# EmbersArc/SCpp

Hardware: AMD Instinct MI355X
Metric: converged SCvx trajectories/sec (RocketQuat, K=50) at 1/2/4/8 MI355X (higher is better)
Workload: dtype f64

## Files before the change

### __graft_entry__.py

```python
import os
import subprocess
import sys

ROOT = os.path.dirname(os.path.abspath(__file__))
CSRC = os.path.join(ROOT, "scpp_amd", "csrc")
HIP_LIB = os.path.join(ROOT, "scpp_amd", "libscpp_hip.so")
HOST_LIB = os.path.join(ROOT, "scpp_amd", "libscpp_host.so")
EMU_LIB = os.path.join(ROOT, "tests", "emu", "libscpp_emu.so")
LQR_LIB = os.path.join(ROOT, "scpp_amd", "libscpp_lqr.so")
LQR_EMU_LIB = os.path.join(ROOT, "tests", "emu", "libscpp_lqr_emu.so")
LQR_SRC = os.path.join(CSRC, "lqr", "scpp_hip_lqr.cpp")
TILE_PROBE_SRC = os.path.join(ROOT, "tests", "tile_probe", "tile_probe.cpp")
TILE_PROBE_LIB = os.path.join(ROOT, "tests", "tile_probe", "libtile_probe.so")
TILE_PROBE_EMU_LIB = os.path.join(ROOT, "tests", "emu", "libtile_probe_emu.so")
SWEEP_PROBE_SRC = os.path.join(ROOT, "tests", "sweep_probe", "sweep_probe.cpp")
SWEEP_PROBE_LIB = os.path.join(ROOT, "tests", "sweep_probe", "libsweep_probe.so")
SWEEP_PROBE_EMU_LIB = os.path.join(ROOT, "tests", "emu", "libsweep_probe_emu.so")
CONE_PROBE_SRC = os.path.join(ROOT, "tests", "cone_probe", "cone_probe.cpp")
CONE_PROBE_LIB = os.path.join(ROOT, "tests", "cone_probe", "libcone_probe.so")
CONE_PROBE_EMU_LIB = os.path.join(ROOT, "tests", "emu", "libcone_probe_emu.so")
PHASE_PROBE_SRC = os.path.join(ROOT, "tests", "phase_probe", "phase_probe.cpp")
PHASE_PROBE_LIB = os.path.join(ROOT, "tests", "phase_probe", "libphase_probe.so")
PHASE_PROBE_MEM_LIB = os.path.join(ROOT, "tests", "phase_probe", "libphase_probe_prevlane_memory.so")
PHASE_PROBE_EMU_LIB = os.path.join(ROOT, "tests", "emu", "libphase_probe_emu.so")
HIP_FP_FLAGS = ["-ffp-contract=on"]


class _BuildLock:

    def __enter__(self):
        import fcntl

        try:
            self.f = open(os.path.join(ROOT, ".build.lock"), "w")
            fcntl.flock(self.f, fcntl.LOCK_EX)
        except OSError:
            self.f = None
        return self

    def __exit__(self, *exc):
        import fcntl

        if self.f is not None:
            fcntl.flock(self.f, fcntl.LOCK_UN)
            self.f.close()
        return False


def _newer(target, sources):
    if not os.path.exists(target):
        return True
    t = os.path.getmtime(target)
    return any(os.path.getmtime(s) > t for s in sources)


def _sources(d, exts):
    out = []
    for base, _, files in os.walk(d):
        out += [os.path.join(base, f) for f in files if f.endswith(exts)]
    return out


def build_hip(force=False):
    srcs = _sources(CSRC, (".h", ".cpp")) + [os.path.join(ROOT, "include", "scpp_hip.h")]
    if force or _newer(HIP_LIB, srcs):
        subprocess.check_call(
            ["hipcc", "--offload-arch=gfx950", "-O3", "-std=c++17", "-fPIC", "-shared", "-x", "hip"] + HIP_FP_FLAGS +
            [os.path.join(CSRC, "scpp_hip.cpp"), "-o", HIP_LIB]
        )
    return HIP_LIB


def build_host(force=False):
    host = os.path.join(ROOT, "scpp_amd", "host")
    if os.path.isdir(host) and os.path.exists(os.path.join(host, "Makefile")):
        with _BuildLock():
            subprocess.check_call(["make", "-s", "-C", host, "all"])


def build_oracle():
    with _BuildLock():
        subprocess.check_call(["make", "-s", "-C", os.path.join(ROOT, "oracle"), "liboracle.so"])


def build_emu(force=False):
    srcs = _sources(CSRC, (".h", ".cpp")) + [os.path.join(ROOT, "tests", "emu", "hip_emu.h")]
    with _BuildLock():
        if force or _newer(EMU_LIB, srcs):
            tmp = EMU_LIB + ".tmp%d" % os.getpid()
            subprocess.check_call(
                ["g++", "-O1", "-std=c++17", "-fPIC", "-DSCPP_HIP_EMU", "-I" + os.path.join(ROOT, "tests", "emu"), "-shared",
                 "-o", tmp, "-x", "c++", os.path.join(CSRC, "scpp_hip.cpp")]
            )
            os.replace(tmp, EMU_LIB)
    return EMU_LIB


def _lqr_sources():
    return _sources(os.path.join(CSRC, "lqr"), (".h", ".cpp")) + [os.path.join(CSRC, f) for f in (
        "common.h", "model_rocketquat.h", "model_lander3dof.h", "model_jacobian_rows.h")] + [os.path.join(ROOT, "include", "scpp_hip_lqr.h")]


def build_lqr(force=False):
    if force or _newer(LQR_LIB, _lqr_sources()):
        subprocess.check_call(
            ["hipcc", "--offload-arch=gfx950", "-O3", "-std=c++17", "-fPIC", "-shared", "-x", "hip"] + HIP_FP_FLAGS + [LQR_SRC, "-o", LQR_LIB]
        )
    return LQR_LIB


def build_lqr_emu(force=False):
    with _BuildLock():
        if force or _newer(LQR_EMU_LIB, _lqr_sources() + [os.path.join(ROOT, "tests", "emu", "hip_emu.h")]):
            tmp = LQR_EMU_LIB + ".tmp%d" % os.getpid()
            subprocess.check_call(
                ["g++", "-O1", "-std=c++17", "-fPIC", "-DSCPP_HIP_EMU", "-I" + os.path.join(ROOT, "tests", "emu"), "-shared",
                 "-o", tmp, "-x", "c++", LQR_SRC]
            )
            os.replace(tmp, LQR_EMU_LIB)
    return LQR_EMU_LIB


def _tile_probe_sources():
    return [TILE_PROBE_SRC] + [os.path.join(CSRC, f) for f in ("tile_engine.h", "ipm_kernel.h", "common.h", "cone_math.h", "constraint_table.h")]


def build_tile_probe(force=False):
    with _BuildLock():
        if force or _newer(TILE_PROBE_LIB, _tile_probe_sources()):
            tmp = TILE_PROBE_LIB + ".tmp%d" % os.getpid()
            subprocess.check_call(
                ["hipcc", "--offload-arch=gfx950", "-O3", "-std=c++17", "-fPIC", "-shared", "-x", "hip"] + HIP_FP_FLAGS + [TILE_PROBE_SRC, "-o", tmp]
            )
            os.replace(tmp, TILE_PROBE_LIB)
    return TILE_PROBE_LIB


def build_tile_probe_emu(force=False):
    with _BuildLock():
        if force or _newer(TILE_PROBE_EMU_LIB, _tile_probe_sources() + [os.path.join(ROOT, "tests", "emu", "hip_emu.h")]):
            tmp = TILE_PROBE_EMU_LIB + ".tmp%d" % os.getpid()
            subprocess.check_call(
                ["g++", "-O1", "-std=c++17", "-fPIC", "-DSCPP_HIP_EMU", "-I" + os.path.join(ROOT, "tests", "emu"), "-shared",
                 "-o", tmp, "-x", "c++", TILE_PROBE_SRC]
            )
            os.replace(tmp, TILE_PROBE_EMU_LIB)
    return TILE_PROBE_EMU_LIB


def _sweep_probe_sources():
    return [SWEEP_PROBE_SRC] + [os.path.join(CSRC, f) for f in ("sweeps.h", "tile_engine.h", "ipm_kernel.h", "common.h", "cone_math.h", "constraint_table.h")]


def build_sweep_probe(force=False):
    with _BuildLock():
        if force or _newer(SWEEP_PROBE_LIB, _sweep_probe_sources()):
            tmp = SWEEP_PROBE_LIB + ".tmp%d" % os.getpid()
            subprocess.check_call(
                ["hipcc", "--offload-arch=gfx950", "-O3", "-std=c++17", "-fPIC", "-shared", "-x", "hip"] + HIP_FP_FLAGS + [SWEEP_PROBE_SRC, "-o", tmp]
            )
            os.replace(tmp, SWEEP_PROBE_LIB)
    return SWEEP_PROBE_LIB


def build_sweep_probe_emu(force=False):
    with _BuildLock():
        if force or _newer(SWEEP_PROBE_EMU_LIB, _sweep_probe_sources() + [os.path.join(ROOT, "tests", "emu", "hip_emu.h")]):
            tmp = SWEEP_PROBE_EMU_LIB + ".tmp%d" % os.getpid()
            subprocess.check_call(
                ["g++", "-O1", "-std=c++17", "-fPIC", "-DSCPP_HIP_EMU", "-I" + os.path.join(ROOT, "tests", "emu"), "-shared",
                 "-o", tmp, "-x", "c++", SWEEP_PROBE_SRC]
            )
            os.replace(tmp, SWEEP_PROBE_EMU_LIB)
    return SWEEP_PROBE_EMU_LIB


def _cone_probe_sources():
    return [CONE_PROBE_SRC] + [os.path.join(CSRC, f) for f in (
        "cone_math.h", "ipm_solve.h", "ipm_kernel.h", "sweeps.h", "tile_engine.h", "common.h", "constraint_table.h")]


def build_cone_probe(force=False):
    with _BuildLock():
        if force or _newer(CONE_PROBE_LIB, _cone_probe_sources()):
            tmp = CONE_PROBE_LIB + ".tmp%d" % os.getpid()
            subprocess.check_call(
                ["hipcc", "--offload-arch=gfx950", "-O3", "-std=c++17", "-fPIC", "-shared", "-x", "hip"] + HIP_FP_FLAGS + [CONE_PROBE_SRC, "-o", tmp]
            )
            os.replace(tmp, CONE_PROBE_LIB)
    return CONE_PROBE_LIB


def build_cone_probe_emu(force=False):
    with _BuildLock():
        if force or _newer(CONE_PROBE_EMU_LIB, _cone_probe_sources() + [os.path.join(ROOT, "tests", "emu", "hip_emu.h")]):
            tmp = CONE_PROBE_EMU_LIB + ".tmp%d" % os.getpid()
            subprocess.check_call(
                ["g++", "-O1", "-std=c++17", "-fPIC", "-DSCPP_HIP_EMU", "-I" + os.path.join(ROOT, "tests", "emu"), "-shared",
                 "-o", tmp, "-x", "c++", CONE_PROBE_SRC]
            )
            os.replace(tmp, CONE_PROBE_EMU_LIB)
    return CONE_PROBE_EMU_LIB


def _phase_probe_sources():
    return [PHASE_PROBE_SRC] + [os.path.join(CSRC, f) for f in (
        "ipm_solve.h", "ipm_kernel.h", "sweeps.h", "tile_engine.h", "common.h", "cone_math.h", "constraint_table.h")]


def _build_phase_probe_hip(lib, defines, force):
    with _BuildLock():
        if force or _newer(lib, _phase_probe_sources()):
            tmp = lib + ".tmp%d" % os.getpid()
            subprocess.check_call(
                ["hipcc", "--offload-arch=gfx950", "-O3", "-std=c++17", "-fPIC", "-shared", "-x", "hip"] + HIP_FP_FLAGS + defines + [PHASE_PROBE_SRC, "-o", tmp]
            )
            os.replace(tmp, lib)
    return lib


def build_phase_probe(force=False):
    return _build_phase_probe_hip(PHASE_PROBE_LIB, [], force)


def build_phase_probe_prevlane_memory(force=False):
    return _build_phase_probe_hip(PHASE_PROBE_MEM_LIB, ["-DRES_PREVLANE_MEMORY=1"], force)


def build_phase_probe_emu(force=False):
    with _BuildLock():
        if force or _newer(PHASE_PROBE_EMU_LIB, _phase_probe_sources() + [os.path.join(ROOT, "tests", "emu", "hip_emu.h")]):
            tmp = PHASE_PROBE_EMU_LIB + ".tmp%d" % os.getpid()
            subprocess.check_call(
                ["g++", "-O1", "-std=c++17", "-fPIC", "-DSCPP_HIP_EMU", "-I" + os.path.join(ROOT, "tests", "emu"), "-shared",
                 "-o", tmp, "-x", "c++", PHASE_PROBE_SRC]
            )
            os.replace(tmp, PHASE_PROBE_EMU_LIB)
    return PHASE_PROBE_EMU_LIB


def build():
    build_hip()
    build_lqr()
    build_host()
    build_oracle()
    build_emu()
    build_lqr_emu()
    build_tile_probe()
    build_tile_probe_emu()
    build_sweep_probe()
    build_sweep_probe_emu()
    build_cone_probe()
    build_cone_probe_emu()
    build_phase_probe()
    build_phase_probe_prevlane_memory()
    build_phase_probe_emu()
    sys.path.insert(0, ROOT)
    import scpp_amd

    scpp_amd.load_library(HIP_LIB)


def smoke():
    sys.path.insert(0, ROOT)
    sys.path.insert(0, os.path.join(ROOT, "tests"))
    import numpy as np
    import scpp_amd
    import oracle_lib

    if not os.path.exists(HIP_LIB):
        build_hip()
    model = scpp_amd.RocketQuat().loadParameters()
    B, K = 4, 50
    x0 = model.randomized_initial_states(B)
    alg = scpp_amd.SCAlgorithm(model, K=K, batch_max=B, device=0, library=os.environ.get("SCPP_HIP_LIBRARY")).initialize()
    alg.solve(x0)
    out = alg.getSolution()
    ref = oracle_lib.sc_batch(K, 20260927, 0, B, nthreads=4, solver=1)
    sx = np.abs(ref["X"]).max(axis=1, keepdims=True)
    su = np.abs(ref["U"]).max(axis=1, keepdims=True)
    relX = float((np.abs(out["X"] - ref["X"]) / np.maximum(sx, 1e-9)).max())
    relU = float((np.abs(out["U"] - ref["U"]) / np.maximum(su, 1e-9)).max())
    assert (out["status"] == 0).all(), out["status"]
    assert (out["sc_iters"] == ref["iters"]).all(), (out["sc_iters"], ref["iters"])
    assert relX < 1e-5 and relU < 1e-5, (relX, relU)
    print(f"smoke ok: relX={relX:.2e} relU={relU:.2e} sc_iters={out['sc_iters'].tolist()} nu={out['nu_norm'].tolist()}")
    alg.ctx.close()
    import lqr_reference

    if not os.path.exists(LQR_LIB):
        build_lqr()
    trk = scpp_amd.LQRTracker(model, out["X"], out["U"], out["sigma"], library=os.environ.get("SCPP_LQR_LIBRARY"))
    assert trk.n_ok == B * K, (trk.n_ok, trk.status)
    Ks = lqr_reference.scipy_gain(0, out["X"][0, 0], out["U"][0, 0], model.flow_params(nondimensionalize=False), trk.Q, trk.R)
    gk = float(np.abs(trk.gains[0, 0] - Ks).max() / np.abs(Ks).max())
    fl = trk.track(x0)
    assert gk < 1e-6 and fl["n_finite"] == B and all(np.isfinite(fl[k]).all() for k in ("x", "u", "err1")), (gk, fl)
    print(f"smoke ok (lqr): {trk.n_ok} gains, node 0 vs scipy {gk:.2e}, {int(fl['steps'].sum())} tracked plant steps, final error / initial error {(fl['err1'] / fl['err0']).round(3).tolist()}")
    trk.close()
    valg = scpp_amd.SCvxAlgorithm(model, K=K, batch_max=4, device=0, library=os.environ.get("SCPP_HIP_LIBRARY")).initialize()
    xs = model.randomized_initial_states(6)
    nconv = valg.solveStream(xs, slots=4, pools=2)
    so = valg.getStreamSolution()
    assert (so["status"] == 0).all() and (so["instance"] == np.arange(6)).all() and nconv == int(so["converged"].sum())
    ov = oracle_lib.SCvx(K=K)
    ov.randomize(20260927, 0)
    ov.set_solver(1)
    assert ov.solve() == 0
    mv = ov.meta()
    Xo, Uo, _ = ov.iterate(-1)
    assert so["converged"][0] == mv["converged"] == 1
    same_path = so["sc_iters"][0] == mv["iterations"] and so["solves"][0] == mv["solves"]
    rx = float(np.abs(so["X"][0] - Xo).max() / np.abs(Xo).max())
    assert rx < (1e-4 if same_path else 5e-2), (rx, same_path)
    print(f"smoke ok (scvx stream): converged {nconv}/6, iterations {so['sc_iters'].tolist()}, solves {so['solves'].tolist()}, relX vs oracle {rx:.2e}")
    valg.ctx.close()
    m2 = scpp_amd.Rocket2D().loadParameters()
    m2.p.constrain_initial_final = False
    mpc = scpp_amd.MPCAlgorithm(m2, batch_max=4, device=0, library=os.environ.get("SCPP_HIP_LIBRARY")).initialize()
    xm = m2.randomized_initial_states(4)
    mpc.setInitialState(xm)
    mpc.setFinalState(m2.p.x_final)
    assert mpc.solve() == 4
    mo = mpc.getSolution()
    o = oracle_lib.MPC()
    for b in range(4):
        r = o.solve(xm[b], kind=1)
        assert r["status"] == 0 and mo["iters"][b] == r["iters"], (b, mo["iters"][b], r["iters"])
        assert np.abs(mo["U"][b] - r["U"]).max() <= 1e-8 * np.abs(r["U"]).max()
    print(f"smoke ok (mpc): iterations {mo['iters'].tolist()}")


if __name__ == "__main__":
    build()
    print("build ok")
```

### scpp_amd/csrc/sweeps.h

```cpp
#pragma once
#include "tile_engine.h"

namespace scpp
{
namespace ipm
{

#ifndef IPM_PRIO_FACTOR
#define IPM_PRIO_FACTOR 1
#endif
#ifndef IPM_PRIO_SUBST
#define IPM_PRIO_SUBST 2
#endif
#if defined(SCPP_HIP_EMU)
#define SET_PRIO(p)
#else
#define SET_PRIO(p) __builtin_amdgcn_s_setprio(p)
#endif
#ifndef SWEEP_PREFETCH
#define SWEEP_PREFETCH 2
#endif
#ifndef SWEEPS_INLINE
#define SWEEP_FN static __device__ __attribute__((noinline, disable_tail_calls))
#else
#define SWEEP_FN __device__ inline __attribute__((always_inline))
#endif

__device__ inline LDSP double *uniformLds(LDSP double *p)
{
#ifdef SCPP_HIP_EMU
    return p;
#else
    return (LDSP double *)(unsigned long long)(unsigned)__builtin_amdgcn_readfirstlane((unsigned)(unsigned long long)p);
#endif
}
__device__ inline Ctx uniformCtx(const LDSP Ctx *cin)
{
    Ctx c;
    c.segl = uniformLds(cin->segl);
    c.K = uniformInt(cin->K);
    c.lane = threadIdx.x;
    c.pitch = uniformInt(cin->pitch);
    c.setup_v0 = uniformInt(cin->setup_v0);
    c.st = uniformPtr(cin->st);
    c.sg = uniformPtr(cin->sg);
    c.dy = uniformPtr(cin->dy);
    c.fac = uniformPtr(cin->fac);
    c.sv = uniformPtr(cin->sv);
    c.sx = uniformPtr(cin->sx);
    c.gsave = uniformPtr(cin->gsave);
    c.A = uniformPtr(cin->A);
    c.B = uniformPtr(cin->B);
    c.C = uniformPtr(cin->C);
    c.S = uniformPtr(cin->S);
    c.Z = uniformPtr(cin->Z);
    c.ip = uniformPtr(cin->ip);
    return c;
}
#ifndef IPM_FAC_LD_AUX
#define IPM_FAC_LD_AUX IPM_LD_AUX
#endif
#ifndef IPM_FAC_ST_AUX
#define IPM_FAC_ST_AUX 2
#endif
#ifndef IPM_DD_LD_AUX
#define IPM_DD_LD_AUX IPM_LD_AUX
#endif
template <int LA, int SA>
struct BufT
{
    __amdgpu_buffer_rsrc_t r;
    __device__ double ld(int vo, int so) const { return __builtin_bit_cast(double, __builtin_amdgcn_raw_buffer_load_b64(r, vo, so, LA)); }
    __device__ void st(int vo, int so, double x) const { __builtin_amdgcn_raw_buffer_store_b64(__builtin_bit_cast(u32x2_t, x), r, vo, so, SA); }
};
typedef BufT<IPM_LD_AUX, IPM_ST_AUX> Buf;
typedef BufT<IPM_FAC_LD_AUX, IPM_FAC_ST_AUX> BufFac;
typedef BufT<IPM_DD_LD_AUX, IPM_ST_AUX> BufDd;
template <class B = Buf>
__device__ inline B makeBuf(const double *p, int ndoubles)
{
    return B{__builtin_amdgcn_make_buffer_rsrc(const_cast<double *>(p), 0, ndoubles * 8, 0x00020000)};
}
struct Off4
{
    int v[4];
};
template <class B>
__device__ inline Tile ldTile(const B &b, const Off4 &o, int so)
{
    Tile t;
#pragma unroll
    for (int r = 0; r < 4; r++)
        t.v[r] = b.ld(o.v[r], so);
    return t;
}
template <class B>
__device__ inline void stTile(const B &b, const Off4 &o, int so, const Tile &t)
{
#pragma unroll
    for (int r = 0; r < 4; r++)
        b.st(o.v[r], so, t.v[r]);
}
template <int n>
__device__ inline Off4 offTri(int lane, int base)
{
    const int g = lane >> 4, i = lane & 15;
    Off4 o;
#pragma unroll
    for (int r = 0; r < 4; r++)
    {
        const int row = g + 4 * r;
        o.v[r] = (row < n && i <= row) ? (base + triIdx(row, i)) * 8 : VO_OOB;
    }
    return o;
}
template <int n>
__device__ inline Off4 offTriT(int lane, int base)
{
    const int g = lane >> 4, i = lane & 15;
    Off4 o;
#pragma unroll
    for (int r = 0; r < 4; r++)
    {
        const int a = g + 4 * r;
        o.v[r] = (i < n && a <= i) ? (base + triIdx(i, a)) * 8 : VO_OOB;
    }
    return o;
}
template <int n>
__device__ inline Tile finishTri(const Tile &raw, int lane)
{
    const int g = lane >> 4, i = lane & 15;
    Tile t = raw;
#pragma unroll
    for (int r = 0; r < 4; r++)
        if (4 * r + 3 >= n)
            t.v[r] = (g + 4 * r >= n && g + 4 * r == i) ? 1. : raw.v[r];
    return t;
}
template <int NL>
__device__ inline Off4 offYt(int lane, int base)
{
    const int g = lane >> 4, i = lane & 15;
    Off4 o;
#pragma unroll
    for (int r = 0; r < 4; r++)
        o.v[r] = i < NL ? (base + (g + 4 * r) * NL + i) * 8 : VO_OOB;
    return o;
}
template <int NL>
__device__ inline Off4 offYtT(int lane, int base)
{
    const int g = lane >> 4, i = lane & 15;
    Off4 o;
#pragma unroll
    for (int r = 0; r < 4; r++)
    {
        const int a = g + 4 * r;
        o.v[r] = a < NL ? (base + i * NL + a) * 8 : VO_OOB;
    }
    return o;
}
__device__ inline Off4 offCols(int lane, int n, int base)
{
    const int g = lane >> 4, i = lane & 15;
    Off4 o;
#pragma unroll
    for (int r = 0; r < 4; r++)
        o.v[r] = i < n ? (base + i * 16 + g + 4 * r) * 8 : VO_OOB;
    return o;
}

template <class P>
struct SweepIO
{
    using L = Lay<P>;
    BufFac fac, sv;
    Buf sx;
    BufDd A, B, C;
    __device__ explicit SweepIO(const Ctx &c)
        : fac(makeBuf<BufFac>(c.fac, c.K * L::FACREC)), sv(makeBuf<BufFac>(c.sv, c.K * SVREC)), sx(makeBuf<Buf>(c.sx, c.K * L::XREC)),
          A(makeBuf<BufDd>(c.A, (c.K - 1) * P::NX * P::NX)), B(makeBuf<BufDd>(c.B, (c.K - 1) * P::NX * P::NU)),
          C(makeBuf<BufDd>(c.C, (c.K - 1) * P::NX * P::NU))
    {
    }
    static __device__ int sFac(int k) { return k * (L::FACREC * 8); }
    static __device__ int sSv(int k) { return k * (SVREC * 8); }
    static __device__ int sX(int k) { return k * (L::XREC * 8); }
    static __device__ int sA(int k) { return k * (P::NX * P::NX * 8); }
    static __device__ int sBC(int k) { return k * (P::NX * P::NU * 8); }
};

struct RhsSpec
{
    int n;
};

__device__ inline RhsSpec uniformSpec(const RhsSpec &s)
{
    RhsSpec o;
    o.n = uniformInt(s.n);
    return o;
}

__device__ inline int colKind(const RhsSpec &sp, int i)
{
    if (sp.n == 2)
        return i == 0 ? 1 : (i == 1 ? 2 : 0);
    return i == 0 ? 2 : 0;
}

template <class P>
__device__ inline Off4 offRhsW(const RhsSpec &sp, int lane)
{
    const int g = lane >> 4, i = lane & 15;
    Off4 o;
#pragma unroll
    for (int r = 0; r < 4; r++)
        o.v[r] = colKind(sp, i) == 2 ? (Lay<P>::X_BETA + g + 4 * r) * 8 : VO_OOB;
    return o;
}
template <class P>
__device__ inline Off4 offRhsL(const RhsSpec &sp, int lane)
{
    const int g = lane >> 4, i = lane & 15;
    const int kind = colKind(sp, i);
    Off4 o;
#pragma unroll
    for (int r = 0; r < 4; r++)
    {
        const int row = g + 4 * r;
        o.v[r] = (kind && row < Lay<P>::NL) ? ((kind == 1 ? Lay<P>::X_S : Lay<P>::X_RHO) + row) * 8 : VO_OOB;
    }
    return o;
}
template <class P>
__device__ inline Off4 offSolW(const RhsSpec &sp, int lane)
{
    const int g = lane >> 4, i = lane & 15;
    const int kind = colKind(sp, i);
    Off4 o;
#pragma unroll
    for (int r = 0; r < 4; r++)
        o.v[r] = kind ? ((kind == 1 ? Lay<P>::X_BCW : Lay<P>::X_VW) + g + 4 * r) * 8 : VO_OOB;
    return o;
}
template <class P>
__device__ inline Off4 offSolL(const RhsSpec &sp, int lane)
{
    const int g = lane >> 4, i = lane & 15;
    const int kind = colKind(sp, i);
    Off4 o;
#pragma unroll
    for (int r = 0; r < 4; r++)
    {
        const int row = g + 4 * r;
        o.v[r] = (kind && row < Lay<P>::NL) ? ((kind == 1 ? Lay<P>::X_BCL : Lay<P>::X_VL) + row) * 8 : VO_OOB;
    }
    return o;
}
__device__ inline Tile rhsLSign(const RhsSpec &sp, int lane, const Tile &t)
{
    const int i = lane & 15;
    if (colKind(sp, i) == 1)
    {
        Tile o;
#pragma unroll
        for (int r = 0; r < 4; r++)
            o.v[r] = -t.v[r];
        return o;
    }
    return t;
}

template <int NC>
__device__ inline constexpr bool colIsBorder(int c)
{
    return NC == 2 && c == 0;
}
template <class P, int NC>
struct VCols
{
    using L = Lay<P>;
    int rw[NC], rl[NC], solW[NC], solL[NC], colL[NC], colS[NC];
    __device__ explicit VCols(int lane)
    {
        const int e = vElem(lane);
        const bool st0 = (lane & 3) == 0;
#pragma unroll
        for (int c = 0; c < NC; c++)
        {
            const bool border = colIsBorder<NC>(c);
            rw[c] = border ? VO_OOB : (L::X_BETA + e) * 8;
            rl[c] = e < L::NL ? ((border ? L::X_S : L::X_RHO) + e) * 8 : VO_OOB;
            solW[c] = st0 ? ((border ? L::X_BCW : L::X_VW) + e) * 8 : VO_OOB;
            solL[c] = (st0 && e < L::NL) ? ((border ? L::X_BCL : L::X_VL) + e) * 8 : VO_OOB;
            colL[c] = (c * 16 + e) * 8;
            colS[c] = st0 ? (c * 16 + e) * 8 : VO_OOB;
        }
    }
    __device__ static double rlSign(int c, double v) { return colIsBorder<NC>(c) ? -v : v; }
};

__device__ inline Tile tileSub(const Tile &a, const Tile &b)
{
    Tile t;
#pragma unroll
    for (int r = 0; r < 4; r++)
        t.v[r] = a.v[r] - b.v[r];
    return t;
}
__device__ inline Tile tileAdd(const Tile &a, const Tile &b)
{
    Tile t;
#pragma unroll
    for (int r = 0; r < 4; r++)
        t.v[r] = a.v[r] + b.v[r];
    return t;
}

struct HRaw
{
    double e2, cc, wcol, wrow[4], hs[4];
};
struct HsLane
{
    int idx[4];
    Off4 off;
};
template <class P>
__device__ inline HsLane hsLane(int lane)
{
    const int g = lane >> 4, i = lane & 15;
    HsLane h;
#pragma unroll
    for (int r = 0; r < 4; r++)
    {
        h.idx[r] = hsIndex<P>(g + 4 * r, i);
        h.off.v[r] = h.idx[r] >= 0 ? (Lay<P>::X_HS + h.idx[r]) * 8 : VO_OOB;
    }
    return h;
}
template <class P>
__device__ inline HRaw loadHRaw(const SweepIO<P> &io, const HsLane &hl, int k, int lane)
{
    using L = Lay<P>;
    const int g = lane >> 4, i = lane & 15;
    const int sk = io.sX(k);
    HRaw h;
    h.e2 = io.sx.ld(L::X_HC * 8, sk);
    h.cc = io.sx.ld((L::X_HC + 1) * 8, sk);
    h.wcol = io.sx.ld((L::X_WBT + i) * 8, sk);
#pragma unroll
    for (int r = 0; r < 4; r++)
    {
        h.wrow[r] = io.sx.ld((L::X_WBT + g + 4 * r) * 8, sk);
        h.hs[r] = io.sx.ld(hl.off.v[r], sk);
    }
    return h;
}
template <class P>
__device__ inline Tile buildHTile(const HRaw &h, const HsLane &hl, int k, int K, int lane, bool scvx)
{
    const int g = lane >> 4, i = lane & 15;
    const unsigned fm = Lay<P>::fixedMask(k, K);
    Tile t;
#pragma unroll
    for (int r = 0; r < 4; r++)
    {
        const int row = g + 4 * r;
        double v = h.e2 * ((row == i ? 1. : 0.) - h.cc * h.wrow[r] * h.wcol);
        if (scvx && (row < P::NXV || i < P::NXV))
            v = 0.;
        v += h.hs[r];
        if ((fm & (1u << row)) || (fm & (1u << i)))
            v = (row == i) ? 1. : 0.;
        t.v[r] = v;
    }
    return t;
}
template <class P>
__device__ inline int varColumn(int j)
{
    using L = Lay<P>;
    if constexpr (L::IDENTITY_MAPS)
        return j < P::NXV ? j : (j < L::NVU ? j - P::NXV : 0);
    else
        return j < P::NXV ? P::XMAP[j] : (j < L::NVU ? P::UMAP[j - P::NXV] : 0);
}
template <class P>
struct OffMt
{
    Off4 a, b;
};
template <class P>
__device__ inline OffMt<P> offMt(int lane)
{
    using L = Lay<P>;
    const int g = lane >> 4, i = lane & 15;
    OffMt<P> o;
#pragma unroll
    for (int r = 0; r < 4; r++)
    {
        const int j = g + 4 * r;
        o.a.v[r] = (i < L::NL && j < P::NXV) ? (i * P::NX + varColumn<P>(j)) * 8 : VO_OOB;
        o.b.v[r] = (i < L::NL && j >= P::NXV && j < L::NVU) ? (i * P::NU + varColumn<P>(j)) * 8 : VO_OOB;
    }
    return o;
}
template <class P>
__device__ inline Tile loadMtRaw(const SweepIO<P> &io, const OffMt<P> &o, int k)
{
    Tile t;
#pragma unroll
    for (int r = 0; r < 4; r++)
    {
        if (4 * r + 3 < P::NXV)
            t.v[r] = io.A.ld(o.a.v[r], io.sA(k));
        else if (4 * r >= P::NXV)
            t.v[r] = (4 * r < Lay<P>::NVU) ? io.B.ld(o.b.v[r], io.sBC(k)) : 0.;
        else
            t.v[r] = io.A.ld(o.a.v[r], io.sA(k)) + io.B.ld(o.b.v[r], io.sBC(k));
    }
    return t;
}
__device__ inline Tile finishMt(const Tile &raw, unsigned fm, int lane)
{
    const int g = lane >> 4;
    Tile t;
#pragma unroll
    for (int r = 0; r < 4; r++)
        t.v[r] = (fm & (1u << (g + 4 * r))) ? 0. : -raw.v[r];
    return t;
}
template <class P>
__device__ inline Off4 offN(int lane)
{
    using L = Lay<P>;
    const int g = lane >> 4, i = lane & 15;
    Off4 o;
#pragma unroll
    for (int r = 0; r < 4; r++)
    {
        const int row = g + 4 * r;
        o.v[r] = (i >= P::NXV && i < L::NVU && row < L::NL) ? (row * P::NU + varColumn<P>(i)) * 8 : VO_OOB;
    }
    return o;
}
template <class P>
__device__ inline Tile finishN(const Tile &raw, unsigned fmn, int lane)
{
    using L = Lay<P>;
    const int g = lane >> 4, i = lane & 15;
    Tile t;
#pragma unroll
    for (int r = 0; r < 4; r++)
    {
        const int row = g + 4 * r;
        double v = 0.;
        if (row < L::NL && !(fmn & (1u << i)))
            v = i < P::NXV ? (row == varColumn<P>(i) ? 1. : 0.) : -raw.v[r];
        t.v[r] = v;
    }
    return t;
}
template <class P>
__device__ inline Off4 offNt(int lane)
{
    using L = Lay<P>;
    const int g = lane >> 4, i = lane & 15;
    Off4 o;
#pragma unroll
    for (int r = 0; r < 4; r++)
    {
        const int a = g + 4 * r;
        o.v[r] = (i < L::NL && a >= P::NXV && a < L::NVU) ? (i * P::NU + varColumn<P>(a)) * 8 : VO_OOB;
    }
    return o;
}
template <class P>
__device__ inline Tile loadNtRaw(const SweepIO<P> &io, const Off4 &o, int k)
{
    Tile t = tileZero();
#pragma unroll
    for (int r = 0; r < 4; r++)
    {
        if (4 * r + 3 < P::NXV || 4 * r >= Lay<P>::NVU)
            continue;
        t.v[r] = io.C.ld(o.v[r], io.sBC(k));
    }
    return t;
}
template <class P>
__device__ inline Tile finishNt(const Tile &raw, unsigned fmn, int lane)
{
    using L = Lay<P>;
    const int g = lane >> 4, i = lane & 15;
    Tile t;
#pragma unroll
    for (int r = 0; r < 4; r++)
    {
        const int a = g + 4 * r;
        double v = 0.;
        if (i < L::NL && !(fmn & (1u << a)))
            v = a < P::NXV ? (varColumn<P>(a) == i ? 1. : 0.) : -raw.v[r];
        t.v[r] = v;
    }
    return t;
}

struct FactorRest
{
    Tile mt, n, rl, rwn;
    double einv;
};
template <class P>
struct FactorOffs
{
    OffMt<P> mt;
    Off4 n, rl, rw, cols, triV, triL, triVT, triLT, yt;
    int einv;
};

template <class P, int NCV>
SWEEP_FN void factorSweepFused(const LDSP Ctx *cin, TileShared &sh, const RhsSpec &spin)
{
    EMU_PHASE("factorSweepFused");
    using L = Lay<P>;
    constexpr int NL = L::NL;
    const Ctx c = uniformCtx(cin);
    const RhsSpec sp = uniformSpec(spin);
    const int lane = c.lane, K = c.K;
    const int g = lane >> 4, i = lane & 15;
    const bool scvx = c.ip[IP_SCVX] != 0.;
    if (IPM_PRIO_FACTOR != IPM_PRIO_LANE)
        SET_PRIO(IPM_PRIO_FACTOR);
    const double dual_reg = scvx ? 1e-9 : 0.;
    const SweepIO<P> io(c);
    FactorOffs<P> o;
    o.mt = offMt<P>(lane);
    o.n = offN<P>(lane);
    o.rl = offRhsL<P>(sp, lane);
    o.rw = offRhsW<P>(sp, lane);
    o.cols = offCols(lane, sp.n, 0);
    o.triV = offTri<NV>(lane, L::FAC_LI);
    o.triL = offTri<NL>(lane, L::FAC_TI);
    o.triVT = offTriT<NV>(lane, L::FAC_LI);
    o.triLT = offTriT<NL>(lane, L::FAC_TI);
    o.yt = offYt<NL>(lane, L::FAC_YT);
    o.einv = i < NL ? (L::X_EINV + i) * 8 : VO_OOB;
#ifdef IPM_PROFILE
    double pf0 = 0., pf1 = 0., pfA = 0., pfC = 0., pfT = 0., pfL = 0., pfH = 0., pfZ = 0.;
    const long long tfs = clock64();
    long long tstage = tfs;
#endif
    constexpr bool VEC = NCV > 0;
    constexpr int NC = VEC ? NCV : 1;
    const VCols<P, NC> vc(lane);
    Tile Z = tileZero(), G = VEC ? tileZero() : ldTile(io.sx, o.rw, io.sX(0));
    double Gv[NC];
#pragma unroll
    for (int q = 0; q < NC; q++)
        Gv[q] = VEC ? io.sx.ld(vc.rw[q], io.sX(0)) : 0.;
    const HsLane hl = hsLane<P>(lane);
    struct Early
    {
        Tile mt;
        double einv;
        HRaw h;
    };
    auto loadEarly = [&](int k) {
        const int ks = k < K - 1 ? k : K - 2;
        Early e;
        e.mt = loadMtRaw<P>(io, o.mt, ks);
        e.einv = io.sx.ld(o.einv, io.sX(ks));
        e.h = loadHRaw<P>(io, hl, k, lane);
        return e;
    };
    auto stage = [&](int k, const Early &cur, Early &nxt) -> bool {
        const int ks = k < K - 1 ? k : K - 2, kn = k + 1 < K ? k + 1 : k;
        const Tile cn = ldTile(io.C, o.n, io.sBC(ks));
        Tile crl, crwn;
        double vrl[NC], vrwn[NC];
        if constexpr (VEC)
        {
#pragma unroll
            for (int q = 0; q < NC; q++)
            {
                vrl[q] = io.sx.ld(vc.rl[q], io.sX(ks));
                vrwn[q] = io.sx.ld(vc.rw[q], io.sX(ks + 1));
            }
        }
        else
        {
            crl = ldTile(io.sx, o.rl, io.sX(ks));
            crwn = ldTile(io.sx, o.rw, io.sX(ks + 1));
        }
        nxt = loadEarly(kn);
        LOADS_ISSUED();
#ifdef IPM_PROFILE
        const long long tfl = clock64();
        pfL += double(tfl - tstage);
#endif
        Tile Phi = buildHTile<P>(cur.h, hl, k, K, lane, scvx);
#ifdef IPM_PROFILE
        const long long tfh = clock64();
        pfH += double(tfh - tfl);
#endif
        if (k > 0)
            Phi = tileAdd(Phi, mm(Z, Z));
#ifdef IPM_PROFILE
        const long long tf0 = clock64();
        pfZ += double(tf0 - tfh);
        pfA += double(tf0 - tstage);
#endif
#if INVCHOL_TRANSPOSED
        const Tile Lit = invCholFactorT<NV>(Phi, lane);
#ifdef IPM_PROFILE
        const long long tf1 = clock64();
        pf0 += double(tf1 - tf0);
#endif
        stTile(io.fac, o.triVT, io.sFac(k), Lit);
#else
        const Tile Li = INVCHOL<NV>(Phi, sh, lane);
#ifdef IPM_PROFILE
        const long long tf1 = clock64();
        pf0 += double(tf1 - tf0);
#endif
        stTile(io.fac, o.triV, io.sFac(k), Li);
        const Tile Lit = transposeTile(Li, sh, lane);
#endif
        Tile a;
        double va[NC];
        if constexpr (VEC)
        {
#pragma unroll
            for (int q = 0; q < NC; q++)
            {
                va[q] = mv(Lit, Gv[q]);
                io.sv.st(vc.colS[q], io.sSv(k), va[q]);
            }
        }
        else
        {
            a = mm(Lit, G);
            stTile(io.sv, o.cols, io.sSv(k), a);
        }
        if (k == K - 1)
            return false;
        const unsigned fm = L::fixedMask(k, K), fmn = L::fixedMask(k + 1, K);
        const Tile Yt = mm(Lit, finishMt(cur.mt, fm, lane));
        stTile(io.fac, o.yt, io.sFac(k), Yt);
        Tile Th = mm(Yt, Yt);
#pragma unroll
        for (int r = 0; r < 4; r++)
        {
            const int row = g + 4 * r;
            if (row == i)
                Th.v[r] = (row < NL) ? Th.v[r] + cur.einv + dual_reg : 1.;
        }
#ifdef IPM_PROFILE
        const long long tf2 = clock64();
        pfC += double(tf2 - tf1);
#endif
#if INVCHOL_TRANSPOSED
        const Tile Tit = invCholFactorT<NL>(Th, lane);
#ifdef IPM_PROFILE
        tstage = clock64();
        pf1 += double(tstage - tf2);
#endif
        stTile(io.fac, o.triLT, io.sFac(k), Tit);
#else
        const Tile Ti = INVCHOL<NL>(Th, sh, lane);
#ifdef IPM_PROFILE
        tstage = clock64();
        pf1 += double(tstage - tf2);
#endif
        stTile(io.fac, o.triL, io.sFac(k), Ti);
        const Tile Tit = transposeTile(Ti, sh, lane);
#endif
        Z = mm(Tit, finishN<P>(cn, fmn, lane));
        if constexpr (VEC)
        {
#pragma unroll
            for (int q = 0; q < NC; q++)
            {
                const double vgl = VCols<P, NC>::rlSign(q, vrl[q]) - mv(Yt, va[q]);
                const double vcc = mv(Tit, vgl);
                io.sv.st(vc.colS[q], io.sSv(k) + NRHS_MAX * 16 * 8, vcc);
                Gv[q] = vrwn[q] + mv(Z, vcc);
            }
        }
        else
        {
            const Tile gl = tileSub(rhsLSign(sp, lane, crl), mm(Yt, a));
            const Tile cc = mm(Tit, gl);
            stTile(io.sv, o.cols, io.sSv(k) + NRHS_MAX * 16 * 8, cc);
            G = tileAdd(crwn, mm(Z, cc));
        }
#ifdef IPM_PROFILE
        {
            const long long tft = clock64();
            pfT += double(tft - tstage);
            pfA += double(tft - tstage);
            tstage = tft;
        }
#endif
        return true;
    };
    Early e0 = loadEarly(0), e1;
    for (int k = 0; k < K; k += 2)
    {
        if (!stage(k, e0, e1))
            break;
        if (!stage(k + 1, e1, e0))
            break;
    }
#ifdef IPM_PROFILE
    if (lane == 0)
    {
        sh.prof[0] += pf0;
        sh.prof[1] += pf1;
        sh.prof[4] += pfA;
        sh.prof[5] += pfC;
        sh.prof[6] += pfT;
        sh.prof[7] += pfL;
        sh.prof[8] += pfH;
        sh.prof[9] += pfZ;
        sh.prof[2] += double(clock64() - tfs);
        sh.prof[3] += 1.;
    }
#endif
    if (IPM_PRIO_FACTOR != IPM_PRIO_LANE)
        SET_PRIO(IPM_PRIO_LANE);
    WAVE_SYNC();
}

struct FwdIn
{
    Tile lit, yt, tit, ti, n, rl, rwn;
};
template <class P>
struct FwdOffs
{
    Off4 lit, yt, tit, ti, n, rl, rw, cols;
};
template <class P>
__device__ inline FwdIn loadFwdIn(const SweepIO<P> &io, const FwdOffs<P> &o, int k, int K)
{
    const int ks = k < K - 1 ? k : K - 2;
    FwdIn f;
    f.lit = ldTile(io.fac, o.lit, io.sFac(k));
    f.yt = ldTile(io.fac, o.yt, io.sFac(ks));
    f.tit = ldTile(io.fac, o.tit, io.sFac(ks));
    f.ti = ldTile(io.fac, o.ti, io.sFac(ks));
    f.n = ldTile(io.C, o.n, io.sBC(ks));
    f.rl = ldTile(io.sx, o.rl, io.sX(ks));
    f.rwn = ldTile(io.sx, o.rw, io.sX(ks + 1));
    return f;
}
template <class P>
SWEEP_FN void fwdSweep(const LDSP Ctx *cin, const RhsSpec &spin)
{
    EMU_PHASE("fwdSweep");
    using L = Lay<P>;
    constexpr int NL = L::NL;
    const Ctx c = uniformCtx(cin);
    const RhsSpec sp = uniformSpec(spin);
    const int lane = c.lane, K = c.K;
    const SweepIO<P> io(c);
    FwdOffs<P> o;
    o.lit = offTriT<NV>(lane, L::FAC_LI);
    o.yt = offYt<NL>(lane, L::FAC_YT);
    o.tit = offTriT<NL>(lane, L::FAC_TI);
    o.ti = offTri<NL>(lane, L::FAC_TI);
    o.n = offN<P>(lane);
    o.rl = offRhsL<P>(sp, lane);
    o.rw = offRhsW<P>(sp, lane);
    o.cols = offCols(lane, sp.n, 0);
    Tile G = ldTile(io.sx, o.rw, io.sX(0));
    auto stage = [&](int k, const FwdIn &cur) -> bool {
        const Tile a = mm(finishTri<NV>(cur.lit, lane), G);
        stTile(io.sv, o.cols, io.sSv(k), a);
        if (k == K - 1)
            return false;
        const Tile gl = tileSub(rhsLSign(sp, lane, cur.rl), mm(cur.yt, a));
        const Tile cc = mm(finishTri<NL>(cur.tit, lane), gl);
        stTile(io.sv, o.cols, io.sSv(k) + NRHS_MAX * 16 * 8, cc);
        G = tileAdd(cur.rwn, mm(finishN<P>(cur.n, L::fixedMask(k + 1, K), lane), mm(finishTri<NL>(cur.ti, lane), cc)));
        return true;
    };
    auto clampK = [&](int k) { return k < K ? k : K - 1; };
#if SWEEP_PREFETCH == 1
    FwdIn b0 = loadFwdIn<P>(io, o, 0, K), b1;
    for (int k = 0; k < K; k += 2)
    {
        b1 = loadFwdIn<P>(io, o, clampK(k + 1), K);
        LOADS_ISSUED();
        if (!stage(k, b0))
            break;
        b0 = loadFwdIn<P>(io, o, clampK(k + 2), K);
        LOADS_ISSUED();
        if (!stage(k + 1, b1))
            break;
    }
#else
    FwdIn b0 = loadFwdIn<P>(io, o, 0, K), b1 = loadFwdIn<P>(io, o, clampK(1), K), b2;
    for (int k = 0; k < K; k += 3)
    {
        b2 = loadFwdIn<P>(io, o, clampK(k + 2), K);
        LOADS_ISSUED();
        if (!stage(k, b0))
            break;
        b0 = loadFwdIn<P>(io, o, clampK(k + 3), K);
        LOADS_ISSUED();
        if (!stage(k + 1, b1))
            break;
        b1 = loadFwdIn<P>(io, o, clampK(k + 4), K);
        LOADS_ISSUED();
        if (!stage(k + 2, b2))
            break;
    }
#endif
    WAVE_SYNC();
}

struct BwdIn
{
    Tile nt, tit, ti, y, li, cs, as;
};
template <class P>
struct BwdOffs
{
    Off4 nt, tit, ti, y, li, cols, solW, solL;
};
template <class P>
__device__ inline BwdIn loadBwdIn(const SweepIO<P> &io, const BwdOffs<P> &o, int k, int K)
{
    const int ks = k < K - 1 ? k : K - 2;
    BwdIn b;
    b.li = ldTile(io.fac, o.li, io.sFac(k));
    b.as = ldTile(io.sv, o.cols, io.sSv(k));
    b.nt = loadNtRaw<P>(io, o.nt, ks);
    b.tit = ldTile(io.fac, o.tit, io.sFac(ks));
    b.ti = ldTile(io.fac, o.ti, io.sFac(ks));
    b.y = ldTile(io.fac, o.y, io.sFac(ks));
    b.cs = ldTile(io.sv, o.cols, io.sSv(ks) + NRHS_MAX * 16 * 8);
    return b;
}
template <class P>
SWEEP_FN void bwdSweep(const LDSP Ctx *cin, const RhsSpec &spin)
{
    EMU_PHASE("bwdSweep");
    using L = Lay<P>;
    constexpr int NL = L::NL;
    const Ctx c = uniformCtx(cin);
    const RhsSpec sp = uniformSpec(spin);
    const int lane = c.lane, K = c.K;
    const SweepIO<P> io(c);
    BwdOffs<P> o;
    o.nt = offNt<P>(lane);
    o.tit = offTriT<NL>(lane, L::FAC_TI);
    o.ti = offTri<NL>(lane, L::FAC_TI);
    o.y = offYtT<NL>(lane, L::FAC_YT);
    o.li = offTri<NV>(lane, L::FAC_LI);
    o.cols = offCols(lane, sp.n, 0);
    o.solW = offSolW<P>(sp, lane);
    o.solL = offSolL<P>(sp, lane);
// ... 262 lines not shown
```

Baseline: 6499.

## Software-pipeline factor sweep stages: build next Hessian tile early, place loads between

Restructures the per-stage factorization sweep so that the next stage's H tile and the Z*Z update into Phi are built at the end of the current stage, and the next stage's loads are issued in the middle of the stage behind AMDGPU sched_barrier fences. The aim is to overlap global/LDS load latency and the independent H-tile construction with the serial inverse-Cholesky chain. It also rewrites buildHTile's masking as selects and pins tiles in registers with empty asm. The cost is higher register pressure and a more rigid compiler schedule, with the old path still available behind a compile-time flag.

```diff
diff --git a/__graft_entry__.py b/__graft_entry__.py
--- a/__graft_entry__.py
+++ b/__graft_entry__.py
@@ -16,6 +16,9 @@
 SWEEP_PROBE_SRC = os.path.join(ROOT, "tests", "sweep_probe", "sweep_probe.cpp")
 SWEEP_PROBE_LIB = os.path.join(ROOT, "tests", "sweep_probe", "libsweep_probe.so")
 SWEEP_PROBE_EMU_LIB = os.path.join(ROOT, "tests", "emu", "libsweep_probe_emu.so")
+SWEEP_PROBE_SCHEDULE_LIB = [os.path.join(ROOT, "tests", "sweep_probe", "libsweep_probe_schedule%d.so" % s) for s in (0, 1)]
+SWEEP_PROBE_SCHEDULE_EMU_LIB = [os.path.join(ROOT, "tests", "emu", "libsweep_probe_schedule%d_emu.so" % s) for s in (0, 1)]
+EMU_SCHEDULE_LIB = [os.path.join(ROOT, "tests", "emu", "libscpp_emu_schedule%d.so" % s) for s in (0, 1)]
 CONE_PROBE_SRC = os.path.join(ROOT, "tests", "cone_probe", "cone_probe.cpp")
 CONE_PROBE_LIB = os.path.join(ROOT, "tests", "cone_probe", "libcone_probe.so")
 CONE_PROBE_EMU_LIB = os.path.join(ROOT, "tests", "emu", "libcone_probe_emu.so")
@@ -83,17 +86,25 @@
         subprocess.check_call(["make", "-s", "-C", os.path.join(ROOT, "oracle"), "liboracle.so"])
 
 
+def _build_emu(lib, defines, force):
+    srcs = _sources(CSRC, (".h", ".cpp")) + [os.path.join(ROOT, "tests", "emu", "hip_emu.h")]
+    with _BuildLock():
+        if force or _newer(lib, srcs):
+            tmp = lib + ".tmp%d" % os.getpid()
+            subprocess.check_call(
+                ["g++", "-O1", "-std=c++17", "-fPIC", "-DSCPP_HIP_EMU", "-I" + os.path.join(ROOT, "tests", "emu"), "-shared"] + defines +
+                ["-o", tmp, "-x", "c++", os.path.join(CSRC, "scpp_hip.cpp")]
+            )
+            os.replace(tmp, lib)
+    return lib
+
+
 def build_emu(force=False):
-    srcs = _sources(CSRC, (".h", ".cpp")) + [os.path.join(ROOT, "tests", "emu", "hip_emu.h")]
-    with _BuildLock():
-        if force or _newer(EMU_LIB, srcs):
-            tmp = EMU_LIB + ".tmp%d" % os.getpid()
-            subprocess.check_call(
-                ["g++", "-O1", "-std=c++17", "-fPIC", "-DSCPP_HIP_EMU", "-I" + os.path.join(ROOT, "tests", "emu"), "-shared",
-                 "-o", tmp, "-x", "c++", os.path.join(CSRC, "scpp_hip.cpp")]
-            )
-            os.replace(tmp, EMU_LIB)
-    return EMU_LIB
+    return _build_emu(EMU_LIB, [], force)
+
+
+def build_emu_schedule(schedule, force=False):
+    return _build_emu(EMU_SCHEDULE_LIB[schedule], ["-DFACTOR_STAGE_SCHEDULE=%d" % schedule], force)
 
 
 def _lqr_sources():
@@ -152,27 +163,51 @@
     return [SWEEP_PROBE_SRC] + [os.path.join(CSRC, f) for f in ("sweeps.h", "tile_engine.h", "ipm_kernel.h", "common.h", "cone_math.h", "constraint_table.h")]
 
 
+def _build_sweep_probe_hip(lib, defines, force):
+    with _BuildLock():
+        if force or _newer(lib, _sweep_probe_sources()):
+            tmp = lib + ".tmp%d" % os.getpid()
+            subprocess.check_call(
+                ["hipcc", "--offload-arch=gfx950", "-O3", "-std=c++17", "-fPIC", "-shared", "-x", "hip"] + HIP_FP_FLAGS + defines + [SWEEP_PROBE_SRC, "-o", tmp]
+            )
+            os.replace(tmp, lib)
+    return lib
+
+
+def _build_sweep_probe_emu(lib, defines, force):
+    with _BuildLock():
+        if force or _newer(lib, _sweep_probe_sources() + [os.path.join(ROOT, "tests", "emu", "hip_emu.h")]):
+            tmp = lib + ".tmp%d" % os.getpid()
+            subprocess.check_call(
+                ["g++", "-O1", "-std=c++17", "-fPIC", "-DSCPP_HIP_EMU", "-I" + os.path.join(ROOT, "tests", "emu"), "-shared"] + defines +
+                ["-o", tmp, "-x", "c++", SWEEP_PROBE_SRC]
+            )
+            os.replace(tmp, lib)
+    return lib
+
+
 def build_sweep_probe(force=False):
-    with _BuildLock():
-        if force or _newer(SWEEP_PROBE_LIB, _sweep_probe_sources()):
-            tmp = SWEEP_PROBE_LIB + ".tmp%d" % os.getpid()
-            subprocess.check_call(
-                ["hipcc", "--offload-arch=gfx950", "-O3", "-std=c++17", "-fPIC", "-shared", "-x", "hip"] + HIP_FP_FLAGS + [SWEEP_PROBE_SRC, "-o", tmp]
-            )
-            os.replace(tmp, SWEEP_PROBE_LIB)
-    return SWEEP_PROBE_LIB
+    return _build_sweep_probe_hip(SWEEP_PROBE_LIB, [], force)
 
 
 def build_sweep_probe_emu(force=False):
-    with _BuildLock():
-        if force or _newer(SWEEP_PROBE_EMU_LIB, _sweep_probe_sources() + [os.path.join(ROOT, "tests", "emu", "hip_emu.h")]):
-            tmp = SWEEP_PROBE_EMU_LIB + ".tmp%d" % os.getpid()
-            subprocess.check_call(
-                ["g++", "-O1", "-std=c++17", "-fPIC", "-DSCPP_HIP_EMU", "-I" + os.path.join(ROOT, "tests", "emu"), "-shared",
-                 "-o", tmp, "-x", "c++", SWEEP_PROBE_SRC]
-            )
-            os.replace(tmp, SWEEP_PROBE_EMU_LIB)
-    return SWEEP_PROBE_EMU_LIB
+    return _build_sweep_probe_emu(SWEEP_PROBE_EMU_LIB, [], force)
+
+
+def build_sweep_probe_schedule0(force=False):
+    return _build_sweep_probe_hip(SWEEP_PROBE_SCHEDULE_LIB[0], ["-DFACTOR_STAGE_SCHEDULE=0"], force)
+
+
+def build_sweep_probe_schedule0_emu(force=False):
+    return _build_sweep_probe_emu(SWEEP_PROBE_SCHEDULE_EMU_LIB[0], ["-DFACTOR_STAGE_SCHEDULE=0"], force)
+
+
+def build_sweep_probe_schedule1(force=False):
+    return _build_sweep_probe_hip(SWEEP_PROBE_SCHEDULE_LIB[1], ["-DFACTOR_STAGE_SCHEDULE=1"], force)
+
+
+def build_sweep_probe_schedule1_emu(force=False):
+    return _build_sweep_probe_emu(SWEEP_PROBE_SCHEDULE_EMU_LIB[1], ["-DFACTOR_STAGE_SCHEDULE=1"], force)
 
 
 def _cone_probe_sources():
@@ -250,6 +285,12 @@
     build_tile_probe_emu()
     build_sweep_probe()
     build_sweep_probe_emu()
+    build_sweep_probe_schedule0()
+    build_sweep_probe_schedule0_emu()
+    build_sweep_probe_schedule1()
+    build_sweep_probe_schedule1_emu()
+    build_emu_schedule(0)
+    build_emu_schedule(1)
     build_cone_probe()
     build_cone_probe_emu()
     build_phase_probe()
diff --git a/scpp_amd/csrc/sweeps.h b/scpp_amd/csrc/sweeps.h
--- a/scpp_amd/csrc/sweeps.h
+++ b/scpp_amd/csrc/sweeps.h
@@ -19,6 +19,21 @@
 #endif
 #ifndef SWEEP_PREFETCH
 #define SWEEP_PREFETCH 2
+#endif
+#ifndef FACTOR_STAGE_SCHEDULE
+#define FACTOR_STAGE_SCHEDULE 1
+#endif
+#ifndef FACTOR_LOADS_BETWEEN
+#define FACTOR_LOADS_BETWEEN 1
+#endif
+#if defined(SCPP_HIP_EMU)
+#define LOADS_NOT_ABOVE()
+#define LOADS_NOT_BELOW()
+#define STAGE_END()
+#else
+#define STAGE_END() __builtin_amdgcn_sched_barrier(0)
+#define LOADS_NOT_ABOVE() __builtin_amdgcn_sched_barrier(0x006)
+#define LOADS_NOT_BELOW() __builtin_amdgcn_sched_barrier(0x00E)
 #endif
 #ifndef SWEEPS_INLINE
 #define SWEEP_FN static __device__ __attribute__((noinline, disable_tail_calls))
@@ -319,6 +334,17 @@
     return t;
 }
 
+__device__ inline void pinTile(Tile &t)
+{
+#ifndef SCPP_HIP_EMU
+#pragma unroll
+    for (int r = 0; r < 4; r++)
+        asm volatile("" : "+v"(t.v[r]));
+#else
+    (void)t;
+#endif
+}
+
 struct HRaw
 {
     double e2, cc, wcol, wrow[4], hs[4];
@@ -370,11 +396,17 @@
     {
         const int row = g + 4 * r;
         double v = h.e2 * ((row == i ? 1. : 0.) - h.cc * h.wrow[r] * h.wcol);
+#if FACTOR_STAGE_SCHEDULE
+        v = (scvx && (row < P::NXV || i < P::NXV)) ? 0. : v;
+        v += h.hs[r];
+        v = (fm & ((1u << row) | (1u << i))) != 0 ? ((row == i) ? 1. : 0.) : v;
+#else
         if (scvx && (row < P::NXV || i < P::NXV))
             v = 0.;
         v += h.hs[r];
         if ((fm & (1u << row)) || (fm & (1u << i)))
             v = (row == i) ? 1. : 0.;
+#endif
         t.v[r] = v;
     }
     return t;
@@ -555,9 +587,15 @@
     long long tstage = tfs;
 #endif
     constexpr bool VEC = NCV > 0;
+    constexpr bool LOADS_BETWEEN = FACTOR_STAGE_SCHEDULE && FACTOR_LOADS_BETWEEN && NCV == 1;
     constexpr int NC = VEC ? NCV : 1;
     const VCols<P, NC> vc(lane);
-    Tile Z = tileZero(), G = VEC ? tileZero() : ldTile(io.sx, o.rw, io.sX(0));
+#if FACTOR_STAGE_SCHEDULE
+    Tile Phi;
+#else
+    Tile Z = tileZero();
+#endif
+    Tile G = VEC ? tileZero() : ldTile(io.sx, o.rw, io.sX(0));
     double Gv[NC];
 #pragma unroll
     for (int q = 0; q < NC; q++)
@@ -577,31 +615,61 @@
         e.h = loadHRaw<P>(io, hl, k, lane);
         return e;
     };
-    auto stage = [&](int k, const Early &cur, Early &nxt) -> bool {
-        const int ks = k < K - 1 ? k : K - 2, kn = k + 1 < K ? k + 1 : k;
-        const Tile cn = ldTile(io.C, o.n, io.sBC(ks));
-        Tile crl, crwn;
+    struct Rest
+    {
+        Tile cn, crl, crwn;
         double vrl[NC], vrwn[NC];
+    };
+    auto loadRest = [&](int k) {
+        const int ks = k < K - 1 ? k : K - 2;
+        Rest r;
+        r.cn = ldTile(io.C, o.n, io.sBC(ks));
         if constexpr (VEC)
         {
 #pragma unroll
             for (int q = 0; q < NC; q++)
             {
-                vrl[q] = io.sx.ld(vc.rl[q], io.sX(ks));
-                vrwn[q] = io.sx.ld(vc.rw[q], io.sX(ks + 1));
+                r.vrl[q] = io.sx.ld(vc.rl[q], io.sX(ks));
+                r.vrwn[q] = io.sx.ld(vc.rw[q], io.sX(ks + 1));
             }
+            r.crl = r.crwn = tileZero();
         }
         else
         {
-            crl = ldTile(io.sx, o.rl, io.sX(ks));
-            crwn = ldTile(io.sx, o.rw, io.sX(ks + 1));
-        }
-        nxt = loadEarly(kn);
-        LOADS_ISSUED();
-#ifdef IPM_PROFILE
-        const long long tfl = clock64();
-        pfL += double(tfl - tstage);
-#endif
+            r.crl = ldTile(io.sx, o.rl, io.sX(ks));
+            r.crwn = ldTile(io.sx, o.rw, io.sX(ks + 1));
+#pragma unroll
+            for (int q = 0; q < NC; q++)
+                r.vrl[q] = r.vrwn[q] = 0.;
+        }
+        return r;
+    };
+    auto stage = [&](int k, Early &cur, Early &nxt, Rest &rc, Rest &rn) -> bool {
+        const int kn = k + 1 < K ? k + 1 : k;
+#ifdef IPM_PROFILE
+        long long tfl = tstage;
+#endif
+        if constexpr (!LOADS_BETWEEN)
+        {
+            rc = loadRest(k);
+            nxt = loadEarly(kn);
+#if FACTOR_STAGE_SCHEDULE
+            LOADS_NOT_BELOW();
+#else
+            LOADS_ISSUED();
+#endif
+#ifdef IPM_PROFILE
+            tfl = clock64();
+            pfL += double(tfl - tstage);
+#endif
+        }
+#if FACTOR_STAGE_SCHEDULE
+        Tile Z;
+#ifdef IPM_PROFILE
+        const long long tf0 = clock64();
+        pfA += double(tf0 - tstage);
+#endif
+#else
         Tile Phi = buildHTile<P>(cur.h, hl, k, K, lane, scvx);
 #ifdef IPM_PROFILE
         const long long tfh = clock64();
@@ -614,6 +682,7 @@
         pfZ += double(tf0 - tfh);
         pfA += double(tf0 - tstage);
 #endif
+#endif
 #if INVCHOL_TRANSPOSED
         const Tile Lit = invCholFactorT<NV>(Phi, lane);
 #ifdef IPM_PROFILE
@@ -632,26 +701,68 @@
 #endif
         Tile a;
         double va[NC];
-        if constexpr (VEC)
-        {
-#pragma unroll
-            for (int q = 0; q < NC; q++)
+        auto savedColumn = [&] {
+            if constexpr (VEC)
             {
-                va[q] = mv(Lit, Gv[q]);
-                io.sv.st(vc.colS[q], io.sSv(k), va[q]);
+#pragma unroll
+                for (int q = 0; q < NC; q++)
+                {
+                    va[q] = mv(Lit, Gv[q]);
+                    io.sv.st(vc.colS[q], io.sSv(k), va[q]);
+                }
             }
-        }
-        else
-        {
-            a = mm(Lit, G);
-            stTile(io.sv, o.cols, io.sSv(k), a);
-        }
+            else
+            {
+                a = mm(Lit, G);
+                stTile(io.sv, o.cols, io.sSv(k), a);
+            }
+        };
+#if !FACTOR_STAGE_SCHEDULE
+        savedColumn();
+#endif
         if (k == K - 1)
+        {
+#if FACTOR_STAGE_SCHEDULE
+            savedColumn();
+#endif
             return false;
+        }
         const unsigned fm = L::fixedMask(k, K), fmn = L::fixedMask(k + 1, K);
         const Tile Yt = mm(Lit, finishMt(cur.mt, fm, lane));
         stTile(io.fac, o.yt, io.sFac(k), Yt);
         Tile Th = mm(Yt, Yt);
+#if FACTOR_STAGE_SCHEDULE
+        savedColumn();
+#ifdef IPM_PROFILE
+        const long long tfh0 = clock64();
+#endif
+        Tile Hn;
+        if constexpr (LOADS_BETWEEN)
+        {
+            LOADS_NOT_ABOVE();
+            rn = loadRest(kn);
+            nxt = loadEarly(kn);
+            LOADS_NOT_BELOW();
+#ifdef IPM_PROFILE
+            const long long tfl1 = clock64();
+            pfL += double(tfl1 - tfh0);
+            pfH -= double(tfl1 - tfh0);
+#endif
+        }
+        else
+        {
+            Hn = buildHTile<P>(nxt.h, hl, kn, K, lane, scvx);
+            pinTile(Hn);
+        }
+        Tile Nk = finishN<P>(rc.cn, fmn, lane);
+        pinTile(Nk);
+#ifdef IPM_PROFILE
+        const long long tfh1 = clock64();
+        pfH += double(tfh1 - tfh0);
+        pfA += double(tfh1 - tfh0);
+        pfC -= double(tfh1 - tfh0);
+#endif
+#endif
 #pragma unroll
         for (int r = 0; r < 4; r++)
         {
@@ -679,25 +790,54 @@
         stTile(io.fac, o.triL, io.sFac(k), Ti);
         const Tile Tit = transposeTile(Ti, sh, lane);
 #endif
-        Z = mm(Tit, finishN<P>(cn, fmn, lane));
+#if FACTOR_STAGE_SCHEDULE
+        Z = mm(Tit, Nk);
+#else
+        Z = mm(Tit, finishN<P>(rc.cn, fmn, lane));
+#endif
+#if FACTOR_STAGE_SCHEDULE
+#ifdef IPM_PROFILE
+        const long long tfz0 = clock64();
+#endif
+#ifdef IPM_PROFILE
+        long long tfz1 = tfz0;
+#endif
+        if constexpr (LOADS_BETWEEN)
+        {
+            Hn = buildHTile<P>(nxt.h, hl, kn, K, lane, scvx);
+#ifdef IPM_PROFILE
+            tfz1 = clock64();
+            pfH += double(tfz1 - tfz0);
+#endif
+        }
+        Phi = tileAdd(Hn, mm(Z, Z));
+#ifdef IPM_PROFILE
+        const long long tfz2 = clock64();
+        pfZ += double(tfz2 - tfz1);
+        pfT -= double(tfz2 - tfz0);
+#endif
+#endif
         if constexpr (VEC)
         {
 #pragma unroll
             for (int q = 0; q < NC; q++)
             {
-                const double vgl = VCols<P, NC>::rlSign(q, vrl[q]) - mv(Yt, va[q]);
+                const double vgl = VCols<P, NC>::rlSign(q, rc.vrl[q]) - mv(Yt, va[q]);
                 const double vcc = mv(Tit, vgl);
                 io.sv.st(vc.colS[q], io.sSv(k) + NRHS_MAX * 16 * 8, vcc);
-                Gv[q] = vrwn[q] + mv(Z, vcc);
+                Gv[q] = rc.vrwn[q] + mv(Z, vcc);
             }
         }
         else
         {
-            const Tile gl = tileSub(rhsLSign(sp, lane, crl), mm(Yt, a));
+            const Tile gl = tileSub(rhsLSign(sp, lane, rc.crl), mm(Yt, a));
             const Tile cc = mm(Tit, gl);
             stTile(io.sv, o.cols, io.sSv(k) + NRHS_MAX * 16 * 8, cc);
-            G = tileAdd(crwn, mm(Z, cc));
-        }
+            G = tileAdd(rc.crwn, mm(Z, cc));
+        }
+#if FACTOR_STAGE_SCHEDULE
+        STAGE_END();
+#endif
 #ifdef IPM_PROFILE
         {
             const long long tft = clock64();
@@ -709,11 +849,20 @@
         return true;
     };
     Early e0 = loadEarly(0), e1;
+    Rest r0, r1;
+#if FACTOR_STAGE_SCHEDULE
+    if constexpr (LOADS_BETWEEN)
+    {
+        r0 = loadRest(0);
+        LOADS_ISSUED();
+    }
+    Phi = buildHTile<P>(e0.h, hl, 0, K, lane, scvx);
+#endif
     for (int k = 0; k < K; k += 2)
     {
-        if (!stage(k, e0, e1))
-            break;
-        if (!stage(k + 1, e1, e0))
+        if (!stage(k, e0, e1, r0, r1))
+            break;
+        if (!stage(k + 1, e1, e0, r1, r0))
             break;
     }
 #ifdef IPM_PROFILE
```

Result: no change. 6542, median of 6 (+0.7%).
